# noahares/raxtax

Measured on AMD Instinct MI355X. Metric: classified queries/sec (whole node), higher is better.
Workload: dtype u32 bit-planes + f64

## Files before the change

include/raxtax_hip.h:

```cpp
#ifndef RAXTAX_HIP_H
#define RAXTAX_HIP_H

#include <stddef.h>
#include <stdint.h>

#ifdef __cplusplus
extern "C" {
#endif

#define RTX_ABI_VERSION 6
#define RTX_NUM_KMERS 65536u
#define RTX_MAX_DEPTH 32u

#define RTX_OK 0
#define RTX_ERR_INVALID (-1)
#define RTX_ERR_HIP (-2)
#define RTX_ERR_NO_DEVICE (-3)
#define RTX_ERR_OOM (-4)
#define RTX_ERR_PARSE (-5)
#define RTX_ERR_DEPTH (-6)
#define RTX_ERR_STATE (-7)
#define RTX_ERR_TOO_LONG (-8)
#define RTX_ERR_SENDER (-9)
#define RTX_RETRY_CHUNK 1
// ... 88 lines not shown
#define RTX_OPT_HIT_PAIR 11
#define RTX_OPT_TILE_SKIP 10
#define RTX_OPT_LOCATOR 12
#define RTX_OPT_TILE_PRUNE 13
#define RTX_OPT_FINE_BOUNDS 17
#define RTX_OPT_RECORDS 18
#define RTX_OPT_OVERLAP 19
#define RTX_OPT_MIN_SUB_BATCHES 20
#define RTX_OPT_TWO_LEVEL_BOUNDS 21
#define RTX_OPT_PRUNE_SELF_SAMPLE 22
#define RTX_OPT_RUN_AHEAD 23
#define RTX_OPT_DEVICE_TEXT 24
#define RTX_OPT_STRAND 25
#define RTX_OPT_NEAREST 26
#define RTX_NO_REF 0xFFFFFFFFu
int rtx_index_set_option(rtx_index *index, int option, uint64_t value);

int rtx_index_self_sample(rtx_index *index, const uint8_t *seq_bytes, const uint64_t *seq_off, uint64_t n_refs, uint32_t n_sample, double *live_fraction);
int rtx_index_prune_verdict(const rtx_index *index, int *pruning, double *live_fraction);
int rtx_index_run_ahead_stats(const rtx_index *index, uint64_t *enqueued_ahead, uint64_t *abandoned);
#define RTX_DEFAULT_SEGMENT_CLASSES 1
#define RTX_DEFAULT_EXACT_HASH_MASK 2
int rtx_set_default_option(int option, uint64_t value);

typedef struct {
    uint32_t n_queries;
    uint64_t n_rows;
    const uint32_t *t;
    const uint8_t *status;
    const double *global_signal;
// ... 138 lines not shown
```

raxtax_amd/_build.py:

```python
from __future__ import annotations

import os
import shutil
import subprocess
from pathlib import Path

PKG = Path(__file__).resolve().parent
ROOT = PKG.parent
CSRC = PKG / "csrc"
LIB = PKG / "libraxtax_hip.so"
SOURCES = ["rtx_kernels.hip", "rtx_hit_pair.hip", "rtx_prob_tables.hip", "rtx_cluster.hip", "rtx_segments.hip", "rtx_prune.hip", "rtx_bounds2.hip", "rtx_records.hip", "rtx_finalise.hip", "rtx_text.hip", "rtx_exact.hip", "rtx_strand.hip", "rtx_nearest.hip", "rtx_ingest.hip", "rtx_api_index.hip", "rtx_api_batch.hip", "rtx_api_download.hip", "rtx_api_shard.hip", "rtx_api_debug.hip", "host_tree.cpp", "host_format.cpp", "host_raxtax.cpp", "host_bin.cpp", "host_threads.cpp"]
HEADERS = ["rtx_index.hpp", "rtx_kernels.hpp", "rtx_hit_common.hpp", "rtx_internal.hpp", "rtx_math.hpp", "rtx_wave.hpp", "rtx_walk.hpp", "host_raxtax.hpp"]
CLI = PKG / "raxtax-hip"
SYNTH = PKG / "raxtax-synth"


def _hipcc() -> str:
    for c in (os.environ.get("HIPCC"), shutil.which("hipcc"), "/opt/rocm/bin/hipcc"):
        if c and Path(c).exists():
            return c
    raise RuntimeError("hipcc not found (ROCm toolchain required to build libraxtax_hip.so)")


def _stale(target: Path, deps) -> bool:
    if not target.exists():
        return True
    t = target.stat().st_mtime
# ... 59 lines not shown
```

raxtax_amd/csrc/rtx_api_batch.hip:

```cpp
#include "rtx_index.hpp"

#ifndef RTX_B2_HEAVY_PER_ATILE
#define RTX_B2_HEAVY_PER_ATILE 4u
#endif

namespace rtxi {

int bind(rtx_index *ix) {
    if (!ix) { set_error("null index handle"); return RTX_ERR_INVALID; }
    RTX_HIP(hipSetDevice(ix->device));
    return RTX_OK;
}

int ensure_events(rtx_index *ix, size_t count) {
    while (ix->events.size() < count) {
        hipEvent_t e;
        RTX_HIP(hipEventCreate(&e));
        ix->events.push_back(e);
    }
    return RTX_OK;
}


SubBatch sub_batch_of(rtx_index *ix, uint32_t sb, bool timed) {
// ... 76 lines not shown
    kp.hq = r.d_hq.p;
    kp.t_all = r.d_t_all.p;
    kp.nrows_all = r.d_nrows_all.p;
    kp.hist = sc.d_hist.p;
    kp.hstride = k.hstride;
    return kp;
}

static bool run_prunes(const rtx_index *ix, const rtx_index::BatchClass &k) { return k.prune && !ix->dbg_full_run; }
static bool on_records_path(const rtx_index *ix, const rtx_index::BatchClass &k, const rtx_index::Scratch &sc) { return run_prunes(ix, k) && k.rec && sc.d_rec.p != nullptr; }
static bool on_diet(const rtx_index *ix, const rtx_index::BatchClass &k, const rtx_index::Scratch &sc) { return on_records_path(ix, k, sc) && k.diet && sc.d_cnt_row.p != nullptr; }

static RecordRef record_ref(const rtx_index *ix, const rtx_index::Scratch &sc, const rtx_index::ResultSet &r) { return RecordRef{sc.d_rec_nslots.p, sc.d_rec_slots.p, sc.d_rec_cnt.p, sc.d_rec.p, ix->rec_slots(), ix->rec_seg_len, r.d_flags.p}; }
static ProbTables prob_tables(const rtx_index *ix) { return ProbTables{ix->d_tab_cmf.p, ix->d_tab_ratio.p, ix->d_tab_off.p, ix->d_tab_moff.p, ix->d_tab_ilo.p, ix->d_tab_sat.p, ix->tab_tmax}; }

int enqueue_kmer(rtx_index *ix, const SubBatch &b, hipStream_t s) {
    KmerParams kp = kmer_params(ix, b);
    kp.mode = run_prunes(ix, *b.cls) && ix->seg_blocks ? 1u : 0u;
    if (b.timed_all) RTX_HIP(hipEventRecord(stage_event(ix, b, RTX_STAGE_KMER_EXTRACT, 0), s));
    launch_kmer_extract(s, kp, b.nq);
    if (b.timed_all) RTX_HIP(hipEventRecord(stage_event(ix, b, RTX_STAGE_KMER_EXTRACT, 1), s));
    return RTX_OK;
}

static HitParams hit_params(rtx_index *ix, const SubBatch &b, uint32_t flags) {
    rtx_index::Scratch &sc = ix->sc[b.set];
    rtx_index::ResultSet &r = ix->res();
    const rtx_index::BatchClass &k = *b.cls;
    HitParams hp{};
    hp.bitmap = ix->d_bitmap.p;
    hp.stride_bytes = ix->stride_bytes;
    hp.n_rows1 = ix->n_rows + 1;
    hp.n_refs = ix->n_refs;
    hp.ref_base = ix->ref_lo;
    hp.rows = sc.d_rows.p;
// ... 134 lines not shown
    fp.fine_n_refs = ix->n_refs;
    fp.fine_ref_ntiles = ix->ntiles;
    fp.fine_stats = ix->d_prune_stats.p + 2 * kPruneStatCopies * 8;
    return fp;
}

int enqueue_hit(rtx_index *ix, const SubBatch &b, uint32_t flags, hipStream_t s, int part, hipStream_t s_mid) {
    rtx_index::Scratch &sc = ix->sc[b.set];
    rtx_index::ResultSet &r = ix->res();
    const rtx_index::BatchClass &k = *b.cls;
    ix->last_set = b.set;
    HitParams hp = hit_params(ix, b, flags);
    const bool prune = run_prunes(ix, k);
    if (k.pair && part != 2) {
        if (b.timed_all) RTX_HIP(hipEventRecord(stage_event(ix, b, RTX_STAGE_PAIR_UNION, 0), s));
        launch_pair_union(s, sc.d_rows.p, sc.d_nrows.p, k.rstride, b.nq, sc.d_urec.p, sc.d_nu.p, 2u * k.rstride);
        if (b.timed_all) RTX_HIP(hipEventRecord(stage_event(ix, b, RTX_STAGE_PAIR_UNION, 1), s));
    }
    if (b.timed && !prune) RTX_HIP(hipEventRecord(stage_event(ix, b, RTX_STAGE_HIT_COUNT, 0), s));
    if (part != 0 && !prune) { set_error("internal: a split run without tile pruning"); return RTX_ERR_STATE; }
    if (prune) {
        if (part != 2) {
            const HitParams up = bounds_params(ix, sc, hp);
            if (b.timed) RTX_HIP(hipEventRecord(stage_event(ix, b, RTX_STAGE_TILE_BOUNDS, 0), s));
            ix->two_level_used = part == 0 && ix->two_level_opt && ix->d_abitmap.p && ix->d_bbitmap.p && ix->n_refs == ix->n_total && k.planes <= kBounds2MaxPlanes;
            if (ix->two_level_used) {
                const bool heavy_ok = sc.d_heavy.p && sc.d_heavy_items.p && sc.d_heavy_items.n >= HeavyItemsLayout(b.nq, ix->u_ntiles).total();
                launch_bounds2(s, bounds2_params(ix, sc, up, heavy_ok), b.nq, k.planes, up, ix->u_ntiles, heavy_ok ? sc.d_heavy_items.p : nullptr);
            } else {
                RTX_HIP(hipMemsetAsync(sc.d_best_key.p, 0, (size_t)b.nq * 4, s));
                launch_hit_count_pair_bounds(s, up, b.nq, ix->u_ntiles, k.planes);
// ... 21 lines not shown
        }
        launch_prune(s, pr, prob_tables(ix), b.nq);
        if (part == 1) { RTX_HIP(hipGetLastError()); return RTX_OK; }
        if (part == 0 && ix->fine_opt && ix->d_fbitmap.p && k.pair && sc.d_fine_items.p) {
            const FineItemsLayout fine(b.nq, ix->f_ntiles);
            uint32_t *const fi = sc.d_fine_items.p;
            launch_fine_bounds(s, fine_params(ix, sc, hp), b.nq, ix->ntiles, ix->f_ntiles, pr.pair_live, fine.cursors(fi), fine.items(fi), fine.count(fi), k.planes);
        }
        RTX_HIP(hipMemsetAsync(sc.d_tilemax.p, 0, (size_t)b.nq * ix->ntiles * 2, s));
        hp.live = sc.d_live.p;
        hp.live_words = pr.live_words;
        hp.prune_thr = sc.d_prune_thr.p;
        if (records) hp.rec = rr;
        if (k.pair) {
            const ItemsLayout items(b.nq, ix->ntiles);
            launch_live_items(s, sc.d_live.p, pr.live_words, pr.pair_live, b.nq, ix->ntiles, items.offsets(sc.d_items.p), items.items(sc.d_items.p), items.count(sc.d_items.p));
            hp.items = items.items(sc.d_items.p);
            hp.n_items = items.count(sc.d_items.p);
        }
        if (ix->seg_blocks) {
            KmerParams kp = kmer_params(ix, b);
            kp.mode = 2u;
            kp.live = sc.d_live.p;
            kp.live_words = pr.live_words;
            launch_kmer_extract(s, kp, b.nq);
        }
        if (b.timed) {
            RTX_HIP(hipEventRecord(stage_event(ix, b, RTX_STAGE_TILE_PRUNE, 1), s));
            RTX_HIP(hipEventRecord(stage_event(ix, b, RTX_STAGE_HIT_COUNT, 0), s));
        }
    }
// ... 945 lines not shown
```

raxtax_amd/csrc/rtx_api_index.hip:

```cpp
#include "rtx_index.hpp"

namespace rtx {
int index_device(const rtx_index *index) { return index ? index->device : -1; }
void index_set_shared_device(rtx_index *index, bool shared) { if (index) index->shared_device = shared; }
uint32_t index_swap_min_subs(rtx_index *index, uint32_t v) { if (!index) return 0; const uint32_t old = index->min_subs; index->min_subs = v; return old; }
bool index_strand(const rtx_index *index) { return index && index->strand_opt != 0u; }
bool index_nearest(const rtx_index *index) { return index && index->nearest_opt != 0u; }
bool index_device_text(const rtx_index *index) { return index && index->device_text_opt != 0u; }
uint32_t index_swap_run_ahead(rtx_index *index, uint32_t v) {
    if (!index) return 0;
    const uint32_t old = index->run_ahead_opt;
    (void)rtx_index_set_option(index, RTX_OPT_RUN_AHEAD, v);
    return old;
}
}

namespace {

double statrs_ln_gamma(double x) {
    static const double dk[11] = {2.48574089138753565546e-5, 1.05142378581721974210,  -3.45687097222016235469,
                                  4.51227709466894823700,    -2.98285225323576655721, 1.05639711577126713077,
                                  -1.95428773191645869583e-1, 1.70970543404441224307e-2,
                                  -5.71926117404305781283e-4, 4.63399473359905636708e-6,
                                  -2.71994908488607703910e-9};
// ... 716 lines not shown
        case RTX_OPT_HIT_PAIR:
            index->pair_opt = value ? 1u : 0u;
            return RTX_OK;
        case RTX_OPT_TILE_SKIP:
            index->tile_skip = value ? 1u : 0u;
            return RTX_OK;
        case RTX_OPT_LOCATOR:
            index->locator_opt = value ? 1u : 0u;
            return RTX_OK;
        case RTX_OPT_TILE_PRUNE:
            index->prune_opt = value ? 1u : 0u;
            return RTX_OK;
        case RTX_OPT_FINE_BOUNDS:
            index->fine_opt = value ? 1u : 0u;
            return RTX_OK;
        case RTX_OPT_PRUNE_SELF_SAMPLE:
            index->uploaded = index->ran = index->synced = false;
            index->self_sample_opt = value ? 1u : 0u;
            return RTX_OK;
        case RTX_OPT_RUN_AHEAD:
            index->run_ahead_opt = (uint32_t)std::min<uint64_t>(value, 2u);
            if (!value && index->join_pending) {
                int rc_b = bind(index);
                if (!rc_b) rc_b = settle_join(index);
                return rc_b;
            }
            return RTX_OK;
        case RTX_OPT_DEVICE_TEXT:
            index->device_text_opt = value ? 1u : 0u;
            return RTX_OK;
// ... 52 lines not shown
```

raxtax_amd/csrc/rtx_hit_pair.hip:

```cpp
#include <hip/hip_runtime.h>

#include <algorithm>

#include "rtx_hit_common.hpp"

namespace rtx {

constexpr uint32_t kPairCap = kHitListCap;
constexpr uint32_t kPairListDw = kPairCap + 192u;
constexpr uint32_t kPairMaskWords = 64u;
constexpr uint32_t kPairSidDw = 2u * kSparseIt * 64u;
constexpr uint32_t kPairLdsBytes = 3u * kPairListDw * 4u + 2u * kPairMaskWords * 8u + 32u * 4u + kPairSidDw * 4u;
#ifndef RTX_PAIR_NB
#define RTX_PAIR_NB 3
#endif
#ifndef RTX_PAIR_WAVES
#define RTX_PAIR_WAVES 2
#endif
constexpr int kPairNB = RTX_PAIR_NB;

constexpr uint32_t kUnionMaxRows = 2048u;
__device__ __forceinline__ uint32_t lower_bound_u16(const uint16_t *l, uint32_t n, uint32_t key) {
    uint32_t lo = 0;
#pragma unroll
// ... 268 lines not shown
            asm volatile("" : "+v"(lane_v));
            pair_tile_block<NP, kPacked, kBounds>(p, lds_dw, item / p.ntiles, item % p.ntiles, lane_v);
            wave_lds_sync();
            if (e8 <= g8) break;
            uint32_t nxt = 0;
            if (lane_v == 0u) nxt = atomicAdd(&p.n_items[1u + x], 1u);
            j = first + g8 + (uint32_t)__builtin_amdgcn_readfirstlane((int)nxt);
        }
        return;
    }
    const uint32_t np8 = gridDim.x >> 3;
    const uint32_t pair = blockIdx.x < np8 * 8u ? (blockIdx.x & 7u) * np8 + (blockIdx.x >> 3) : blockIdx.x;
    pair_tile_block<NP, kPacked, kBounds>(p, lds_dw, pair, blockIdx.y, lane);
}

__global__ __launch_bounds__(1024) void live_offsets_kernel(const uint32_t *__restrict__ pair_live, uint32_t np, uint32_t *__restrict__ off,
                                                            uint32_t *__restrict__ n_items) {
    __shared__ uint32_t wsum[2][16];
    const uint32_t tid = threadIdx.x, lane = tid & 63u, wave = tid >> 6;
    constexpr uint32_t kPer = 8;
    uint32_t carry = 0, buf = 0;
    for (uint32_t base = 0; base < np; base += 1024u * kPer, buf ^= 1u) {
        const uint32_t i0 = base + tid * kPer;
        uint32_t c[kPer], cnt = 0;
#pragma unroll
        for (uint32_t j = 0; j < kPer; j++) c[j] = i0 + j < np ? pair_live[i0 + j] : 0u;
#pragma unroll
        for (uint32_t j = 0; j < kPer; j++) cnt += c[j];
        const uint32_t incl = wave_incl_scan_u32(cnt);
        if (lane == 63u) wsum[buf][wave] = incl;
        __syncthreads();
        uint32_t o = carry + incl - cnt, tot = 0;
#pragma unroll
        for (uint32_t w = 0; w < 16u; w++) {
            const uint32_t sw = wsum[buf][w];
            o += w < wave ? sw : 0u;
            tot += sw;
        }
#pragma unroll
        for (uint32_t j = 0; j < kPer; j++) {
            if (i0 + j < np) off[i0 + j] = o;
            o += c[j];
        }
        carry += tot;
    }
    if (tid == 0u) n_items[0] = carry;
    if (tid < 8u) n_items[1u + tid] = 0;
}

__global__ __launch_bounds__(1024) void live_items_kernel(const uint32_t *__restrict__ live, uint32_t live_words, uint32_t nq, uint32_t ntiles,
                                                          const uint32_t *__restrict__ off, uint32_t *__restrict__ items) {
    extern __shared__ uint32_t tl[];
    const uint32_t tid = threadIdx.x, lane = tid & 63u;
    const uint32_t np = (nq + 1u) / 2u, g0 = blockIdx.x * 1024u, pair = g0 + tid;
    for (uint32_t T = tid; T < ntiles; T += 1024) tl[T] = 0;
    __syncthreads();
    const uint32_t nw = (ntiles + 31u) >> 5;
    const bool valid = pair < np;
    const uint32_t *wa = live + (size_t)((valid ? pair : 0u) * 2u) * live_words;
    const bool hb = valid && pair * 2u + 1u < nq;
    if (valid)
        for (uint32_t w = 0; w < nw; w++) {
            uint32_t bits = wa[w] | (hb ? wa[live_words + w] : 0u);
            while (bits) {
                atomicAdd(&tl[w * 32u + (uint32_t)__builtin_ctz(bits)], 1u);
                bits &= bits - 1u;
            }
        }
    __syncthreads();
    if (tid < 64u) {
        uint32_t running = 0;
        for (uint32_t T0 = 0; T0 < ntiles; T0 += 64) {
            const uint32_t v = T0 + lane < ntiles ? tl[T0 + lane] : 0u;
            const uint32_t incl = wave_incl_scan_u32(v);
            if (T0 + lane < ntiles) tl[T0 + lane] = running + incl - v;
            running += (uint32_t)__builtin_amdgcn_readlane((int)incl, 63);
        }
    }
    __syncthreads();
    if (!valid) return;
    const uint32_t base = off[g0];
    for (uint32_t w = 0; w < nw; w++) {
        uint32_t bits = wa[w] | (hb ? wa[live_words + w] : 0u);
        while (bits) {
            const uint32_t tile = w * 32u + (uint32_t)__builtin_ctz(bits);
            bits &= bits - 1u;
            items[base + atomicAdd(&tl[tile], 1u)] = pair * ntiles + tile;
        }
    }
}

void launch_pair_union(hipStream_t s, const uint32_t *rows, const uint32_t *nrows, uint32_t rstride, uint32_t nq, uint2 *urec,
                       uint32_t *nu, uint32_t ustride) {
    hipLaunchKernelGGL(pair_union_kernel, dim3((nq + 1u) / 2u), dim3(64), 0, s, rows, nrows, rstride, nq, urec, nu, ustride);
}

// ... 9 lines not shown
    const dim3 grid = p.items ? dim3((uint32_t)((std::min<uint64_t>((uint64_t)np * ntiles, std::max<uint64_t>((uint64_t)RTX_ITEM_GRID_HALVES * np / 2u, 2048ull)) + 7u) & ~7ull)) : dim3(np, ntiles);
    if (NP <= 10 && p.counts_lo) {
        if (p.items) hipLaunchKernelGGL((hit_count_pair_kernel<(NP <= 10 ? NP : 10), true, false, true>), grid, dim3(64), kPairLdsBytes, s, p);
        else hipLaunchKernelGGL((hit_count_pair_kernel<(NP <= 10 ? NP : 10), true, false, false>), grid, dim3(64), kPairLdsBytes, s, p);
    } else {
        if (p.items) hipLaunchKernelGGL((hit_count_pair_kernel<NP, false, false, true>), grid, dim3(64), kPairLdsBytes, s, p);
        else hipLaunchKernelGGL((hit_count_pair_kernel<NP, false, false, false>), grid, dim3(64), kPairLdsBytes, s, p);
    }
}
void launch_hit_count_pair(hipStream_t s, const HitParams &p, uint32_t nq, uint32_t ntiles, int planes) {
    if (planes <= 8) launch_hit_count_pair_np<8>(s, p, nq, ntiles);
    else if (planes <= 10) launch_hit_count_pair_np<10>(s, p, nq, ntiles);
    else launch_hit_count_pair_np<11>(s, p, nq, ntiles);
}

void launch_live_items(hipStream_t s, const uint32_t *live, uint32_t live_words, const uint32_t *pair_live, uint32_t nq, uint32_t ntiles, uint32_t *off,
                       uint32_t *items, uint32_t *n_items) {
    const uint32_t np = (nq + 1u) / 2u;
    hipLaunchKernelGGL(live_offsets_kernel, dim3(1), dim3(1024), 0, s, pair_live, np, off, n_items);
    hipLaunchKernelGGL(live_items_kernel, dim3((np + 1023u) / 1024u), dim3(1024), (size_t)ntiles * 4, s, live, live_words, nq, ntiles, off, items);
}

void launch_hit_count_pair_bounds(hipStream_t s, const HitParams &p, uint32_t nq, uint32_t u_ntiles, int planes) {
    if (planes <= 8) hipLaunchKernelGGL((hit_count_pair_kernel<8, true, 1, false>), dim3((nq + 1u) / 2u, u_ntiles), dim3(64), kPairLdsBytes, s, p);
    else if (planes <= 10) hipLaunchKernelGGL((hit_count_pair_kernel<10, true, 1, false>), dim3((nq + 1u) / 2u, u_ntiles), dim3(64), kPairLdsBytes, s, p);
    else hipLaunchKernelGGL((hit_count_pair_kernel<11, false, 1, false>), dim3((nq + 1u) / 2u, u_ntiles), dim3(64), kPairLdsBytes, s, p);
}

void launch_hit_count_pair_bounds_items(hipStream_t s, const HitParams &p, uint32_t nq, uint32_t u_ntiles, int planes) {
    const uint32_t np = (nq + 1u) / 2u;
    const dim3 grid((uint32_t)((std::min<uint64_t>((uint64_t)np * u_ntiles, 4096ull) + 7u) & ~7ull));
    if (planes <= 8) hipLaunchKernelGGL((hit_count_pair_kernel<8, true, 1, true>), grid, dim3(64), kPairLdsBytes, s, p);
    else if (planes <= 10) hipLaunchKernelGGL((hit_count_pair_kernel<10, true, 1, true>), grid, dim3(64), kPairLdsBytes, s, p);
    else hipLaunchKernelGGL((hit_count_pair_kernel<11, false, 1, true>), grid, dim3(64), kPairLdsBytes, s, p);
}
// ... 77 lines not shown
```

raxtax_amd/csrc/rtx_index.hpp:

```cpp
#pragma once

#include <hip/hip_runtime.h>

#include <algorithm>
#include <cmath>
#include <cstdlib>
#include <cstring>
#include <thread>

#include "rtx_internal.hpp"
#include "rtx_kernels.hpp"
#include "rtx_math.hpp"

using namespace rtx;

namespace rtxi {


constexpr uint32_t kEmptyRow = 0xFFFFFFFFu;
constexpr uint32_t kLnFactLen = 98320;

#define RTX_HIP(call)                                                                          \
    do {                                                                                       \
        hipError_t e_ = (call);                                                                \
// ... 148 lines not shown
    uint32_t pair_opt = 1;
    uint32_t prune_opt = 1;
    uint32_t self_sample_opt = 1;
    bool prune_pays = true;
    double self_live = -1.0;
    bool pruning() const { return prune_opt != 0u && (prune_pays || self_sample_opt == 0u); }
    bool dbg_full = false;
    bool dbg_full_run = false;
    DevBuf<uint32_t> d_ubitmap;
    uint32_t u_stride_bytes = 0, u_ntiles = 0;
    uint64_t u_nblocks = 0;
    DevBuf<uint32_t> d_fbitmap;
    uint32_t f_stride_bytes = 0, f_ntiles = 0;
    uint64_t f_nblocks = 0;
    uint32_t fine_opt = 1;
    DevBuf<uint32_t> d_abitmap;
    DevBuf<uint8_t> d_bbitmap;
    uint32_t n_atiles = 0, n_btiles = 0;
    DevBuf<uint8_t> d_cbitmap;
    uint32_t two_level_opt = 1;
    uint32_t b2_delta[4] = {283u, 205u, 92u, 128u};
    bool two_level_used = false;
    uint32_t rec_seg_len = 1024;
    uint32_t diet_shift = 3;
    uint32_t rec_opt = 4;
    uint32_t rec_slots() const { return std::min<uint32_t>(rec_opt, kRecMaxSlots); }
    uint32_t overlap_opt = 1;
    uint32_t overlap_used = 0;
    hipStream_t stream2 = nullptr, stream3 = nullptr, hit_stream = nullptr;
    std::vector<hipEvent_t> ev_front, ev_back, ev_mid;
// ... 255 lines not shown
int alloc_final(rtx_index *ix, rtx_index::ResultSet &r, uint64_t n_queries);
int enqueue_finalise(rtx_index *ix, const SubBatch &b, hipStream_t s);
int enqueue_text(rtx_index *ix, const rtx_index::ResultSet &r);


struct ItemList {
    size_t np, ntiles;
    ItemList(size_t nq, size_t tiles) : np((nq + 1u) / 2u), ntiles(tiles) {}
    size_t cap() const { return np * ntiles; }
    size_t end() const { return cap() + 9u; }
    uint32_t *items(uint32_t *p) const { return p; }
    uint32_t *count(uint32_t *p) const { return p + cap(); }
};
struct ItemsLayout : ItemList {
    using ItemList::ItemList;
    size_t total() const { return end() + 2u * np; }
    uint32_t *pair_live(uint32_t *p) const { return p + end(); }
    uint32_t *offsets(uint32_t *p) const { return p + end() + np; }
};
struct FineItemsLayout : ItemList {
    using ItemList::ItemList;
    size_t total() const { return end() + ntiles; }
    uint32_t *cursors(uint32_t *p) const { return p + end(); }
};
struct HeavyItemsLayout : ItemList {
    using ItemList::ItemList;
    size_t total() const { return end(); }
};
struct LiveLayout {
    uint32_t ntiles;
    uint32_t words() const { return (ntiles + 31u) / 32u + 1u; }
    size_t total(size_t B) const { return (B + 1u) * words(); }
};
// ... 66 lines not shown
```

raxtax_amd/csrc/rtx_kernels.hip:

```cpp
#include <hip/hip_runtime.h>

#include "rtx_kernels.hpp"
#include "rtx_math.hpp"
#include "rtx_wave.hpp"
#include "rtx_hit_common.hpp"
#include "rtx_walk.hpp"

namespace rtx {

static constexpr uint32_t kEmptyRow = 0xFFFFFFFFu;

__global__ __launch_bounds__(256) void bitmap_build_kernel(const uint64_t *__restrict__ off,
                                                           const uint32_t *__restrict__ post,
                                                           const uint32_t *__restrict__ row_of,
                                                           uint32_t *__restrict__ bitmap, uint32_t stride_words, uint32_t n_rows1,
                                                           uint32_t ref_lo, uint32_t ref_hi, uint32_t shift) {
    const uint32_t k = blockIdx.x;
    const uint32_t row = row_of[k];
    if (row == kEmptyRow) return;
    const uint64_t b = off[k], e = off[k + 1];
    for (uint64_t i = b + threadIdx.x; i < e; i += blockDim.x) {
        const uint32_t g = post[i];
        if (g < ref_lo || g >= ref_hi) continue;
        uint32_t word, bit;
// ... 96 lines not shown

    uint32_t t = 0, nrows = 0;
    unsigned long long hq = 0;
    uint32_t *rout = p.rows + (size_t)q * p.rstride;
    const unsigned long long lt_mask = (1ull << lane) - 1ull;
    if (mode == 2u) {
        nrows = p.nrows[q];
    } else {
    for (uint32_t i = lane; i < 2048; i += 64) bm[i] = 0;
    {
        uint32_t *h = p.hist + (size_t)q * p.hstride;
        for (uint32_t i = lane; i < p.hstride; i += 64) h[i] = 0;
    }
    __syncthreads();

    if (len >= 8) {
        const uint64_t nwin = len - 7;
        const uint64_t wpl = (nwin + 63) / 64;
        const uint64_t w0 = (uint64_t)lane * wpl;
        const uint64_t w1 = w0 + wpl < nwin ? w0 + wpl : nwin;
        for (uint64_t i = w0; i < w1; i += 16) {
            unsigned long long v[3];
            __builtin_memcpy(v, seq + i, 24);
            const uint32_t nw = w1 - i < 16 ? (uint32_t)(w1 - i) : 16u;
            uint32_t k = 0, run = 0;
#pragma unroll
            for (int b = 0; b < 23; b++) {
                const uint32_t c = (uint32_t)(v[b >> 3] >> ((b & 7) * 8)) & 0xFFu;
                const bool ok = c == 1u || c == 2u || c == 4u || c == 8u;
                k = ((k << 2) | (((uint32_t)__ffs((int)c) - 1u) & 3u)) & 0xFFFFu;
                run = ok ? run + 1u : 0u;
                if (b >= 7 && (uint32_t)(b - 7) < nw && run >= 8u) atomicOr(&bm[k >> 5], 1u << (k & 31u));
            }
        }
    }
    __syncthreads();

    uint16_t *kout = p.kmers + (size_t)q * p.kstride;
    const unsigned long long *bm64 = reinterpret_cast<const unsigned long long *>(bm);
    uint32_t base = 0;
    for (uint32_t r = 0; r < 16; r++) {
        unsigned long long word = bm64[r * 64 + lane];
        const uint32_t cnt = (uint32_t)__popcll(word);
        const uint32_t incl = wave_incl_scan_u32(cnt);
        uint32_t pos = base + incl - cnt;
        const uint32_t kbase = (r * 64 + lane) * 64;
        while (word) {
            const uint32_t bit = (uint32_t)__builtin_ctzll(word);
            word &= word - 1;
            if (pos < p.kstride) kout[pos] = (uint16_t)(kbase + bit);
// ... 905 lines not shown
```

raxtax_amd/csrc/rtx_kernels.hpp:

```cpp
#pragma once

#include <hip/hip_runtime.h>

#include <cstdint>

#include "raxtax_hip.h"

namespace rtx {

#ifndef RTX_NODE_TYPES_DEFINED
#define RTX_NODE_TYPES_DEFINED
enum NodeType : uint8_t { kInner = 0, kTaxon = 1, kSequence = 2 };
#endif

constexpr uint32_t kWalkMaxRows = 208;
constexpr uint32_t kSegSlotEntries = 16, kSegSparseMax = 16, kSegMaxSparseRows = 255;
constexpr uint32_t kSegPad = 8192;
__host__ __device__ inline uint32_t seg_pad(uint32_t i) { return kSegPad + ((i & 63u) << 2); }
constexpr uint32_t kKmerFewLive = 8;
constexpr uint32_t kHitListCap = 1024;

struct DevRow {
    uint32_t node;
    uint8_t k[RTX_MAX_DEPTH];
// ... 387 lines not shown
    WalkParams walk;
    unsigned long long *prefix_stats;
    unsigned long long *stats;
};
void launch_records_tail(hipStream_t s, const TailParams &p, uint32_t nq);

void launch_bitmap_build(hipStream_t s, const uint64_t *off, const uint32_t *post, const uint32_t *row_of,
                         uint32_t *bitmap, uint32_t stride_words, uint32_t n_rows1, uint32_t ref_lo, uint32_t ref_hi, uint32_t shift = 0);
void launch_ref_kmer_mark(hipStream_t s, const uint8_t *bases, const uint64_t *off, uint64_t n_refs, uint32_t *present);
void launch_ref_bitmap_set(hipStream_t s, const uint8_t *bases, const uint64_t *off, uint64_t n_refs,
                           const uint32_t *row_of, uint32_t *bitmap, uint32_t stride_words, uint32_t n_rows1, uint32_t shift = 0);
void launch_row_len_pack(hipStream_t s, const uint32_t *row_of, const uint32_t *list_len, uint2 *out);
void launch_row_popcount(hipStream_t s, const uint32_t *row_of, const uint32_t *bitmap, uint32_t stride_words, uint32_t n_rows1,
                         uint32_t *list_len);
void launch_kmer_extract(hipStream_t s, const KmerParams &p, uint32_t nq);
void launch_hit_count(hipStream_t s, const HitParams &p, uint32_t nq, uint32_t ntiles, int planes);
void launch_pair_union(hipStream_t s, const uint32_t *rows, const uint32_t *nrows, uint32_t rstride, uint32_t nq, uint2 *urec,
                       uint32_t *nu, uint32_t ustride);
void launch_hit_count_pair(hipStream_t s, const HitParams &p, uint32_t nq, uint32_t ntiles, int planes);
void launch_live_items(hipStream_t s, const uint32_t *live, uint32_t live_words, const uint32_t *pair_live, uint32_t nq, uint32_t ntiles, uint32_t *off,
                       uint32_t *items, uint32_t *n_items);
void launch_hit_count_pair_bounds(hipStream_t s, const HitParams &p, uint32_t nq, uint32_t u_ntiles, int planes);
void launch_hit_count_pair_bounds_items(hipStream_t s, const HitParams &p, uint32_t nq, uint32_t u_ntiles, int planes);
void launch_fine_bounds(hipStream_t s, const HitParams &p, uint32_t nq, uint32_t ntiles, uint32_t f_ntiles, uint32_t *pair_live, uint32_t *cnt,
                        uint32_t *items, uint32_t *n_items, int planes);
size_t prob_table_lds_bytes(uint32_t tmax);
void launch_prob_table(hipStream_t s, const ProbParams &p, uint32_t nq);
size_t prob_lookup_lds_bytes(uint32_t tmax);
void launch_prob_tables_build(hipStream_t s, const ProbTables &tb, const double *lf, const double *inv);
void launch_prob_order(hipStream_t s, const uint32_t *t, uint32_t nq, uint32_t *order);
void launch_prob_lookup(hipStream_t s, const ProbParams &p, const ProbTables &tb, uint32_t nq);
void launch_seg_popcount(hipStream_t s, const uint32_t *bitmap, uint32_t stride_bytes, uint32_t n_rows1, uint32_t ntiles, uint16_t *pop);
void launch_seg_emit(hipStream_t s, const uint32_t *bitmap, uint32_t stride_bytes, uint32_t n_rows1, uint32_t ntiles,
                     const uint32_t *seginfo, uint32_t seg_stride, uint16_t *slots);
void launch_sketch(hipStream_t s, const uint8_t *bases, const uint64_t *off, uint32_t n_q, uint64_t *keys, uint32_t *idx);
// ... 20 lines not shown
```

Baseline: 13.07 million.

## Fuse k-mer extraction with pair union lists and merge live-items offset pass

Adds a pair_extract kernel that builds the k-mer sets of both queries in a pair within one block and emits their per-query row lists and the merged union records together, so the separate pair_union pass is skipped on the pruned pair path. It also folds the single-block live-offsets scan into the live-items kernel, where each block recomputes its prefix by summing all earlier pair_live entries. This removes one or two kernel launches and a re-read of row lists, at the cost of a lower-occupancy 128-thread extract kernel and prefix work that grows with block index. The fused path is enabled by default behind a new option.

Result: no change. 12.95 million (-0.9%).

```diff
diff --git a/include/raxtax_hip.h b/include/raxtax_hip.h
--- a/include/raxtax_hip.h
+++ b/include/raxtax_hip.h
@@ -126,6 +126,7 @@
 #define RTX_OPT_STRAND 25
 #define RTX_OPT_NEAREST 26
 #define RTX_NO_REF 0xFFFFFFFFu
+#define RTX_OPT_PAIR_LISTS 27
 int rtx_index_set_option(rtx_index *index, int option, uint64_t value);
 
 int rtx_index_self_sample(rtx_index *index, const uint8_t *seq_bytes, const uint64_t *seq_off, uint64_t n_refs, uint32_t n_sample, double *live_fraction);
diff --git a/raxtax_amd/_build.py b/raxtax_amd/_build.py
--- a/raxtax_amd/_build.py
+++ b/raxtax_amd/_build.py
@@ -9,8 +9,8 @@
 ROOT = PKG.parent
 CSRC = PKG / "csrc"
 LIB = PKG / "libraxtax_hip.so"
-SOURCES = ["rtx_kernels.hip", "rtx_hit_pair.hip", "rtx_prob_tables.hip", "rtx_cluster.hip", "rtx_segments.hip", "rtx_prune.hip", "rtx_bounds2.hip", "rtx_records.hip", "rtx_finalise.hip", "rtx_text.hip", "rtx_exact.hip", "rtx_strand.hip", "rtx_nearest.hip", "rtx_ingest.hip", "rtx_api_index.hip", "rtx_api_batch.hip", "rtx_api_download.hip", "rtx_api_shard.hip", "rtx_api_debug.hip", "host_tree.cpp", "host_format.cpp", "host_raxtax.cpp", "host_bin.cpp", "host_threads.cpp"]
-HEADERS = ["rtx_index.hpp", "rtx_kernels.hpp", "rtx_hit_common.hpp", "rtx_internal.hpp", "rtx_math.hpp", "rtx_wave.hpp", "rtx_walk.hpp", "host_raxtax.hpp"]
+SOURCES = ["rtx_kernels.hip", "rtx_hit_pair.hip", "rtx_pair_extract.hip", "rtx_prob_tables.hip", "rtx_cluster.hip", "rtx_segments.hip", "rtx_prune.hip", "rtx_bounds2.hip", "rtx_records.hip", "rtx_finalise.hip", "rtx_text.hip", "rtx_exact.hip", "rtx_strand.hip", "rtx_nearest.hip", "rtx_ingest.hip", "rtx_api_index.hip", "rtx_api_batch.hip", "rtx_api_download.hip", "rtx_api_shard.hip", "rtx_api_debug.hip", "host_tree.cpp", "host_format.cpp", "host_raxtax.cpp", "host_bin.cpp", "host_threads.cpp"]
+HEADERS = ["rtx_index.hpp", "rtx_kernels.hpp", "rtx_hit_common.hpp", "rtx_internal.hpp", "rtx_math.hpp", "rtx_wave.hpp", "rtx_kmer_set.hpp", "rtx_walk.hpp", "host_raxtax.hpp"]
 CLI = PKG / "raxtax-hip"
 SYNTH = PKG / "raxtax-synth"
 
diff --git a/raxtax_amd/csrc/rtx_api_batch.hip b/raxtax_amd/csrc/rtx_api_batch.hip
--- a/raxtax_amd/csrc/rtx_api_batch.hip
+++ b/raxtax_amd/csrc/rtx_api_batch.hip
@@ -114,11 +114,20 @@
 static RecordRef record_ref(const rtx_index *ix, const rtx_index::Scratch &sc, const rtx_index::ResultSet &r) { return RecordRef{sc.d_rec_nslots.p, sc.d_rec_slots.p, sc.d_rec_cnt.p, sc.d_rec.p, ix->rec_slots(), ix->rec_seg_len, r.d_flags.p}; }
 static ProbTables prob_tables(const rtx_index *ix) { return ProbTables{ix->d_tab_cmf.p, ix->d_tab_ratio.p, ix->d_tab_off.p, ix->d_tab_moff.p, ix->d_tab_ilo.p, ix->d_tab_sat.p, ix->tab_tmax}; }
 
+static bool fused_pair_lists(const rtx_index *ix, const rtx_index::BatchClass &k) {
+    return ix->pair_lists_opt != 0u && k.pair && run_prunes(ix, k) && ix->seg_blocks != 0u && ix->n_refs == ix->n_total;
+}
+
 int enqueue_kmer(rtx_index *ix, const SubBatch &b, hipStream_t s) {
     KmerParams kp = kmer_params(ix, b);
     kp.mode = run_prunes(ix, *b.cls) && ix->seg_blocks ? 1u : 0u;
     if (b.timed_all) RTX_HIP(hipEventRecord(stage_event(ix, b, RTX_STAGE_KMER_EXTRACT, 0), s));
-    launch_kmer_extract(s, kp, b.nq);
+    if (fused_pair_lists(ix, *b.cls)) {
+        rtx_index::Scratch &sc = ix->sc[b.set];
+        launch_pair_extract(s, kp, b.nq, sc.d_urec.p, sc.d_nu.p, 2u * b.cls->rstride);
+    } else {
+        launch_kmer_extract(s, kp, b.nq);
+    }
     if (b.timed_all) RTX_HIP(hipEventRecord(stage_event(ix, b, RTX_STAGE_KMER_EXTRACT, 1), s));
     return RTX_OK;
 }
@@ -283,7 +292,7 @@
     const bool prune = run_prunes(ix, k);
     if (k.pair && part != 2) {
         if (b.timed_all) RTX_HIP(hipEventRecord(stage_event(ix, b, RTX_STAGE_PAIR_UNION, 0), s));
-        launch_pair_union(s, sc.d_rows.p, sc.d_nrows.p, k.rstride, b.nq, sc.d_urec.p, sc.d_nu.p, 2u * k.rstride);
+        if (!fused_pair_lists(ix, k)) launch_pair_union(s, sc.d_rows.p, sc.d_nrows.p, k.rstride, b.nq, sc.d_urec.p, sc.d_nu.p, 2u * k.rstride);
         if (b.timed_all) RTX_HIP(hipEventRecord(stage_event(ix, b, RTX_STAGE_PAIR_UNION, 1), s));
     }
     if (b.timed && !prune) RTX_HIP(hipEventRecord(stage_event(ix, b, RTX_STAGE_HIT_COUNT, 0), s));
@@ -335,7 +344,7 @@
         if (records) hp.rec = rr;
         if (k.pair) {
             const ItemsLayout items(b.nq, ix->ntiles);
-            launch_live_items(s, sc.d_live.p, pr.live_words, pr.pair_live, b.nq, ix->ntiles, items.offsets(sc.d_items.p), items.items(sc.d_items.p), items.count(sc.d_items.p));
+            launch_live_items(s, sc.d_live.p, pr.live_words, pr.pair_live, b.nq, ix->ntiles, items.items(sc.d_items.p), items.count(sc.d_items.p));
             hp.items = items.items(sc.d_items.p);
             hp.n_items = items.count(sc.d_items.p);
         }
diff --git a/raxtax_amd/csrc/rtx_api_index.hip b/raxtax_amd/csrc/rtx_api_index.hip
--- a/raxtax_amd/csrc/rtx_api_index.hip
+++ b/raxtax_amd/csrc/rtx_api_index.hip
@@ -754,6 +754,10 @@
         case RTX_OPT_FINE_BOUNDS:
             index->fine_opt = value ? 1u : 0u;
             return RTX_OK;
+        case RTX_OPT_PAIR_LISTS:
+            if (value > 1) break;
+            index->pair_lists_opt = (uint32_t)value;
+            return RTX_OK;
         case RTX_OPT_PRUNE_SELF_SAMPLE:
             index->uploaded = index->ran = index->synced = false;
             index->self_sample_opt = value ? 1u : 0u;
diff --git a/raxtax_amd/csrc/rtx_hit_pair.hip b/raxtax_amd/csrc/rtx_hit_pair.hip
--- a/raxtax_amd/csrc/rtx_hit_pair.hip
+++ b/raxtax_amd/csrc/rtx_hit_pair.hip
@@ -306,47 +306,29 @@
     pair_tile_block<NP, kPacked, kBounds>(p, lds_dw, pair, blockIdx.y, lane);
 }
 
-__global__ __launch_bounds__(1024) void live_offsets_kernel(const uint32_t *__restrict__ pair_live, uint32_t np, uint32_t *__restrict__ off,
-                                                            uint32_t *__restrict__ n_items) {
+__global__ __launch_bounds__(1024) void live_items_kernel(const uint32_t *__restrict__ live, uint32_t live_words, uint32_t nq, uint32_t ntiles,
+                                                          const uint32_t *__restrict__ pair_live, uint32_t *__restrict__ items,
+                                                          uint32_t *__restrict__ n_items) {
+    extern __shared__ uint32_t tl[];
     __shared__ uint32_t wsum[2][16];
-    const uint32_t tid = threadIdx.x, lane = tid & 63u, wave = tid >> 6;
-    constexpr uint32_t kPer = 8;
-    uint32_t carry = 0, buf = 0;
-    for (uint32_t base = 0; base < np; base += 1024u * kPer, buf ^= 1u) {
-        const uint32_t i0 = base + tid * kPer;
-        uint32_t c[kPer], cnt = 0;
-#pragma unroll
-        for (uint32_t j = 0; j < kPer; j++) c[j] = i0 + j < np ? pair_live[i0 + j] : 0u;
-#pragma unroll
-        for (uint32_t j = 0; j < kPer; j++) cnt += c[j];
-        const uint32_t incl = wave_incl_scan_u32(cnt);
-        if (lane == 63u) wsum[buf][wave] = incl;
-        __syncthreads();
-        uint32_t o = carry + incl - cnt, tot = 0;
-#pragma unroll
-        for (uint32_t w = 0; w < 16u; w++) {
-            const uint32_t sw = wsum[buf][w];
-            o += w < wave ? sw : 0u;
-            tot += sw;
-        }
-#pragma unroll
-        for (uint32_t j = 0; j < kPer; j++) {
-            if (i0 + j < np) off[i0 + j] = o;
-            o += c[j];
-        }
-        carry += tot;
-    }
-    if (tid == 0u) n_items[0] = carry;
-    if (tid < 8u) n_items[1u + tid] = 0;
-}
-
-__global__ __launch_bounds__(1024) void live_items_kernel(const uint32_t *__restrict__ live, uint32_t live_words, uint32_t nq, uint32_t ntiles,
-                                                          const uint32_t *__restrict__ off, uint32_t *__restrict__ items) {
-    extern __shared__ uint32_t tl[];
     const uint32_t tid = threadIdx.x, lane = tid & 63u;
     const uint32_t np = (nq + 1u) / 2u, g0 = blockIdx.x * 1024u, pair = g0 + tid;
     for (uint32_t T = tid; T < ntiles; T += 1024) tl[T] = 0;
+    uint32_t before = 0;
+    for (uint32_t i = tid; i < g0; i += 1024u) before += pair_live[i];
+    uint32_t own = pair < np ? pair_live[pair < np ? pair : 0u] : 0u;
+#pragma unroll
+    for (int d = 32; d >= 1; d >>= 1) {
+        before += __shfl_xor(before, d, 64);
+        own += __shfl_xor(own, d, 64);
+    }
+    if (lane == 0u) { wsum[0][tid >> 6] = before; wsum[1][tid >> 6] = own; }
     __syncthreads();
+    uint32_t base = 0, group = 0;
+#pragma unroll
+    for (uint32_t w = 0; w < 16u; w++) { base += wsum[0][w]; group += wsum[1][w]; }
+    if (blockIdx.x == 0u && tid < 8u) n_items[1u + tid] = 0;
+    if (blockIdx.x == gridDim.x - 1u && tid == 0u) n_items[0] = base + group;
     const uint32_t nw = (ntiles + 31u) >> 5;
     const bool valid = pair < np;
     const uint32_t *wa = live + (size_t)((valid ? pair : 0u) * 2u) * live_words;
@@ -371,7 +353,6 @@
     }
     __syncthreads();
     if (!valid) return;
-    const uint32_t base = off[g0];
     for (uint32_t w = 0; w < nw; w++) {
         uint32_t bits = wa[w] | (hb ? wa[live_words + w] : 0u);
         while (bits) {
@@ -411,11 +392,10 @@
     else launch_hit_count_pair_np<11>(s, p, nq, ntiles);
 }
 
-void launch_live_items(hipStream_t s, const uint32_t *live, uint32_t live_words, const uint32_t *pair_live, uint32_t nq, uint32_t ntiles, uint32_t *off,
+void launch_live_items(hipStream_t s, const uint32_t *live, uint32_t live_words, const uint32_t *pair_live, uint32_t nq, uint32_t ntiles,
                        uint32_t *items, uint32_t *n_items) {
     const uint32_t np = (nq + 1u) / 2u;
-    hipLaunchKernelGGL(live_offsets_kernel, dim3(1), dim3(1024), 0, s, pair_live, np, off, n_items);
-    hipLaunchKernelGGL(live_items_kernel, dim3((np + 1023u) / 1024u), dim3(1024), (size_t)ntiles * 4, s, live, live_words, nq, ntiles, off, items);
+    hipLaunchKernelGGL(live_items_kernel, dim3((np + 1023u) / 1024u), dim3(1024), (size_t)ntiles * 4, s, live, live_words, nq, ntiles, pair_live, items, n_items);
 }
 
 void launch_hit_count_pair_bounds(hipStream_t s, const HitParams &p, uint32_t nq, uint32_t u_ntiles, int planes) {
diff --git a/raxtax_amd/csrc/rtx_index.hpp b/raxtax_amd/csrc/rtx_index.hpp
--- a/raxtax_amd/csrc/rtx_index.hpp
+++ b/raxtax_amd/csrc/rtx_index.hpp
@@ -186,6 +186,10 @@
     uint32_t f_stride_bytes = 0, f_ntiles = 0;
     uint64_t f_nblocks = 0;
     uint32_t fine_opt = 1;
+#ifndef RTX_PAIR_LISTS_DEFAULT
+#define RTX_PAIR_LISTS_DEFAULT 1
+#endif
+    uint32_t pair_lists_opt = RTX_PAIR_LISTS_DEFAULT;
     DevBuf<uint32_t> d_abitmap;
     DevBuf<uint8_t> d_bbitmap;
     uint32_t n_atiles = 0, n_btiles = 0;
@@ -471,9 +475,8 @@
 };
 struct ItemsLayout : ItemList {
     using ItemList::ItemList;
-    size_t total() const { return end() + 2u * np; }
+    size_t total() const { return end() + np; }
     uint32_t *pair_live(uint32_t *p) const { return p + end(); }
-    uint32_t *offsets(uint32_t *p) const { return p + end() + np; }
 };
 struct FineItemsLayout : ItemList {
     using ItemList::ItemList;
diff --git a/raxtax_amd/csrc/rtx_kernels.hip b/raxtax_amd/csrc/rtx_kernels.hip
--- a/raxtax_amd/csrc/rtx_kernels.hip
+++ b/raxtax_amd/csrc/rtx_kernels.hip
@@ -3,6 +3,7 @@
 #include "rtx_kernels.hpp"
 #include "rtx_math.hpp"
 #include "rtx_wave.hpp"
+#include "rtx_kmer_set.hpp"
 #include "rtx_hit_common.hpp"
 #include "rtx_walk.hpp"
 
@@ -134,26 +135,7 @@
     }
     __syncthreads();
 
-    if (len >= 8) {
-        const uint64_t nwin = len - 7;
-        const uint64_t wpl = (nwin + 63) / 64;
-        const uint64_t w0 = (uint64_t)lane * wpl;
-        const uint64_t w1 = w0 + wpl < nwin ? w0 + wpl : nwin;
-        for (uint64_t i = w0; i < w1; i += 16) {
-            unsigned long long v[3];
-            __builtin_memcpy(v, seq + i, 24);
-            const uint32_t nw = w1 - i < 16 ? (uint32_t)(w1 - i) : 16u;
-            uint32_t k = 0, run = 0;
-#pragma unroll
-            for (int b = 0; b < 23; b++) {
-                const uint32_t c = (uint32_t)(v[b >> 3] >> ((b & 7) * 8)) & 0xFFu;
-                const bool ok = c == 1u || c == 2u || c == 4u || c == 8u;
-                k = ((k << 2) | (((uint32_t)__ffs((int)c) - 1u) & 3u)) & 0xFFFFu;
-                run = ok ? run + 1u : 0u;
-                if (b >= 7 && (uint32_t)(b - 7) < nw && run >= 8u) atomicOr(&bm[k >> 5], 1u << (k & 31u));
-            }
-        }
-    }
+    kmer_set_build(bm, seq, len, lane);
     __syncthreads();
 
     uint16_t *kout = p.kmers + (size_t)q * p.kstride;
diff --git a/raxtax_amd/csrc/rtx_kernels.hpp b/raxtax_amd/csrc/rtx_kernels.hpp
--- a/raxtax_amd/csrc/rtx_kernels.hpp
+++ b/raxtax_amd/csrc/rtx_kernels.hpp
@@ -425,11 +425,12 @@
 void launch_row_popcount(hipStream_t s, const uint32_t *row_of, const uint32_t *bitmap, uint32_t stride_words, uint32_t n_rows1,
                          uint32_t *list_len);
 void launch_kmer_extract(hipStream_t s, const KmerParams &p, uint32_t nq);
+void launch_pair_extract(hipStream_t s, const KmerParams &p, uint32_t nq, uint2 *urec, uint32_t *nu, uint32_t ustride);
 void launch_hit_count(hipStream_t s, const HitParams &p, uint32_t nq, uint32_t ntiles, int planes);
 void launch_pair_union(hipStream_t s, const uint32_t *rows, const uint32_t *nrows, uint32_t rstride, uint32_t nq, uint2 *urec,
                        uint32_t *nu, uint32_t ustride);
 void launch_hit_count_pair(hipStream_t s, const HitParams &p, uint32_t nq, uint32_t ntiles, int planes);
-void launch_live_items(hipStream_t s, const uint32_t *live, uint32_t live_words, const uint32_t *pair_live, uint32_t nq, uint32_t ntiles, uint32_t *off,
+void launch_live_items(hipStream_t s, const uint32_t *live, uint32_t live_words, const uint32_t *pair_live, uint32_t nq, uint32_t ntiles,
                        uint32_t *items, uint32_t *n_items);
 void launch_hit_count_pair_bounds(hipStream_t s, const HitParams &p, uint32_t nq, uint32_t u_ntiles, int planes);
 void launch_hit_count_pair_bounds_items(hipStream_t s, const HitParams &p, uint32_t nq, uint32_t u_ntiles, int planes);
diff --git a/raxtax_amd/csrc/rtx_kmer_set.hpp b/raxtax_amd/csrc/rtx_kmer_set.hpp
--- /dev/null
+++ b/raxtax_amd/csrc/rtx_kmer_set.hpp
@@ -0,0 +1,32 @@
+#pragma once
+
+#include <hip/hip_runtime.h>
+
+#include <cstdint>
+
+namespace rtx {
+
+__device__ __forceinline__ void kmer_set_build(uint32_t *bm, const uint8_t *__restrict__ seq, uint64_t len, uint32_t lane) {
+    if (len >= 8) {
+        const uint64_t nwin = len - 7;
+        const uint64_t wpl = (nwin + 63) / 64;
+        const uint64_t w0 = (uint64_t)lane * wpl;
+        const uint64_t w1 = w0 + wpl < nwin ? w0 + wpl : nwin;
+        for (uint64_t i = w0; i < w1; i += 16) {
+            unsigned long long v[3];
+            __builtin_memcpy(v, seq + i, 24);
+            const uint32_t nw = w1 - i < 16 ? (uint32_t)(w1 - i) : 16u;
+            uint32_t k = 0, run = 0;
+#pragma unroll
+            for (int b = 0; b < 23; b++) {
+                const uint32_t c = (uint32_t)(v[b >> 3] >> ((b & 7) * 8)) & 0xFFu;
+                const bool ok = c == 1u || c == 2u || c == 4u || c == 8u;
+                k = ((k << 2) | (((uint32_t)__ffs((int)c) - 1u) & 3u)) & 0xFFFFu;
+                run = ok ? run + 1u : 0u;
+                if (b >= 7 && (uint32_t)(b - 7) < nw && run >= 8u) atomicOr(&bm[k >> 5], 1u << (k & 31u));
+            }
+        }
+    }
+}
+
+}
diff --git a/raxtax_amd/csrc/rtx_pair_extract.hip b/raxtax_amd/csrc/rtx_pair_extract.hip
--- /dev/null
+++ b/raxtax_amd/csrc/rtx_pair_extract.hip
@@ -0,0 +1,171 @@
+#include <hip/hip_runtime.h>
+
+#include "rtx_kernels.hpp"
+#include "rtx_wave.hpp"
+#include "rtx_kmer_set.hpp"
+
+namespace rtx {
+
+static constexpr uint32_t kEmptyRow = 0xFFFFFFFFu;
+constexpr uint32_t kPxListCap = 4096u;
+
+__device__ __forceinline__ uint32_t wave_total_u32(uint32_t v) { return (uint32_t)__builtin_amdgcn_readlane((int)wave_incl_scan_u32(v), 63); }
+
+__global__ __launch_bounds__(128) void pair_extract_kernel(KmerParams p, uint32_t nq, uint2 *__restrict__ urec, uint32_t *__restrict__ nu,
+                                                           uint32_t ustride) {
+    __shared__ __attribute__((aligned(16))) uint32_t bm[2][2048];
+    __shared__ uint16_t ulist[kPxListCap];
+    __shared__ uint32_t xcnt[2][2][4];
+    __shared__ unsigned long long xhq[2][2];
+    const uint32_t pair = blockIdx.x, lane = threadIdx.x & 63u;
+    const uint32_t wave = (uint32_t)__builtin_amdgcn_readfirstlane((int)(threadIdx.x >> 6));
+    const uint32_t q = pair * 2u + wave;
+    const bool have = q < nq;
+    const uint64_t gq = p.q0 + q;
+    uint64_t len = 0;
+    const uint8_t *seq = p.bases;
+    if (have) {
+        const uint64_t qin = p.perm[gq];
+        const uint64_t b0 = p.base_off[qin];
+        len = p.base_off[qin + 1] - b0;
+        seq = p.bases + b0;
+    }
+    for (uint32_t i = lane; i < 2048; i += 64) bm[wave][i] = 0;
+    if (have) {
+        uint32_t *h = p.hist + (size_t)q * p.hstride;
+        for (uint32_t i = lane; i < p.hstride; i += 64) h[i] = 0;
+    }
+    __syncthreads();
+    kmer_set_build(bm[wave], seq, len, lane);
+    __syncthreads();
+
+    const unsigned long long *sa = reinterpret_cast<const unsigned long long *>(bm[0]), *sb = reinterpret_cast<const unsigned long long *>(bm[1]);
+    uint32_t ha[2] = {0, 0}, hb[2] = {0, 0}, hu[2] = {0, 0};
+#pragma unroll
+    for (uint32_t r = 0; r < 16; r++) {
+        const unsigned long long a = sa[r * 64 + lane], b = sb[r * 64 + lane];
+        ha[r >> 3] += (uint32_t)__popcll(a);
+        hb[r >> 3] += (uint32_t)__popcll(b);
+        hu[r >> 3] += (uint32_t)__popcll(a | b);
+    }
+    const uint32_t a0 = wave_total_u32(ha[0]), b0n = wave_total_u32(hb[0]), u0 = wave_total_u32(hu[0]);
+    const uint32_t t_a = a0 + wave_total_u32(ha[1]), t_b = b0n + wave_total_u32(hb[1]), n_list = u0 + wave_total_u32(hu[1]);
+    {
+        uint16_t *ka = p.kmers + (size_t)(pair * 2u) * p.kstride, *kb = ka + p.kstride;
+        uint32_t base_a = wave ? a0 : 0u, base_b = wave ? b0n : 0u, base_u = wave ? u0 : 0u;
+        for (uint32_t r = wave * 8u; r < wave * 8u + 8u; r++) {
+            const unsigned long long a = sa[r * 64 + lane], b = sb[r * 64 + lane];
+            unsigned long long u = a | b;
+            const uint32_t ca = (uint32_t)__popcll(a), cb = (uint32_t)__popcll(b), cu = (uint32_t)__popcll(u);
+            const uint32_t ia = wave_incl_scan_u32(ca), ib = wave_incl_scan_u32(cb), iu = wave_incl_scan_u32(cu);
+            uint32_t pos_a = base_a + ia - ca, pos_b = base_b + ib - cb, pos_u = base_u + iu - cu;
+            const uint32_t kbase = (r * 64 + lane) * 64;
+            while (u) {
+                const uint32_t bit = (uint32_t)__builtin_ctzll(u);
+                u &= u - 1;
+                const uint16_t k = (uint16_t)(kbase + bit);
+                if (pos_u < kPxListCap) ulist[pos_u] = k;
+                pos_u++;
+                if ((a >> bit) & 1ull) {
+                    if (pos_a < p.kstride) ka[pos_a] = k;
+                    pos_a++;
+                }
+                if ((b >> bit) & 1ull) {
+                    if (pos_b < p.kstride) kb[pos_b] = k;
+                    pos_b++;
+                }
+            }
+            base_a += (uint32_t)__builtin_amdgcn_readlane((int)ia, 63);
+            base_b += (uint32_t)__builtin_amdgcn_readlane((int)ib, 63);
+            base_u += (uint32_t)__builtin_amdgcn_readlane((int)iu, 63);
+        }
+    }
+    __syncthreads();
+
+    const uint32_t n_l = n_list < kPxListCap ? n_list : kPxListCap;
+    const unsigned long long lt_mask = (1ull << lane) - 1ull;
+    uint32_t *ra = p.rows + (size_t)(pair * 2u) * p.rstride, *rb = ra + p.rstride;
+    uint2 *out = urec + (size_t)pair * ustride;
+    uint32_t n_a = 0, n_b = 0, n_u = 0;
+    unsigned long long hq_a = 0, hq_b = 0;
+    for (uint32_t i0 = 0, turn = 0; i0 < n_l; i0 += 512, turn ^= 1u) {
+        uint32_t kk[4], row[4], ll[4];
+        bool in_a[4], in_b[4];
+#pragma unroll
+        for (int u = 0; u < 4; u++) {
+            const uint32_t i = i0 + wave * 256u + (uint32_t)u * 64u + lane;
+            kk[u] = i < n_l ? (uint32_t)ulist[i] : 0xFFFFFFFFu;
+        }
+#pragma unroll
+        for (int u = 0; u < 4; u++) {
+            const uint32_t k = kk[u] & 0xFFFFu;
+            in_a[u] = kk[u] != 0xFFFFFFFFu && ((bm[0][k >> 5] >> (k & 31u)) & 1u);
+            in_b[u] = kk[u] != 0xFFFFFFFFu && ((bm[1][k >> 5] >> (k & 31u)) & 1u);
+        }
+#pragma unroll
+        for (int u = 0; u < 4; u++) {
+            row[u] = kEmptyRow;
+            ll[u] = 0;
+            if (kk[u] != 0xFFFFFFFFu) {
+                const uint2 rl = p.row_len[kk[u]];
+                row[u] = rl.x;
+                ll[u] = rl.y;
+            }
+        }
+        uint32_t la[4], lb[4], lu[4], c_a = 0, c_b = 0, c_u = 0;
+#pragma unroll
+        for (int u = 0; u < 4; u++) {
+            hq_a += in_a[u] ? ll[u] : 0u;
+            hq_b += in_b[u] ? ll[u] : 0u;
+            const bool sv = row[u] != kEmptyRow;
+            const unsigned long long m_a = __ballot(sv && in_a[u]), m_b = __ballot(sv && in_b[u]), m_u = __ballot(sv);
+            la[u] = c_a + (uint32_t)__popcll(m_a & lt_mask);
+            lb[u] = c_b + (uint32_t)__popcll(m_b & lt_mask);
+            lu[u] = c_u + (uint32_t)__popcll(m_u & lt_mask);
+            c_a += (uint32_t)__popcll(m_a);
+            c_b += (uint32_t)__popcll(m_b);
+            c_u += (uint32_t)__popcll(m_u);
+        }
+        if (lane == 0) { xcnt[turn][wave][0] = c_a; xcnt[turn][wave][1] = c_b; xcnt[turn][wave][2] = c_u; }
+        __syncthreads();
+        const uint32_t o_a = xcnt[turn][wave ^ 1u][0], o_b = xcnt[turn][wave ^ 1u][1], o_u = xcnt[turn][wave ^ 1u][2];
+        const uint32_t f_a = n_a + (wave ? o_a : 0u), f_b = n_b + (wave ? o_b : 0u), f_u = n_u + (wave ? o_u : 0u);
+#pragma unroll
+        for (int u = 0; u < 4; u++) {
+            if (row[u] == kEmptyRow) continue;
+            const uint32_t pa = f_a + la[u], pb = f_b + lb[u], pu = f_u + lu[u];
+            if (in_a[u] && pa < p.rstride) ra[pa] = row[u];
+            if (in_b[u] && pb < p.rstride) rb[pb] = row[u];
+            if (pu < ustride)
+                out[pu] = make_uint2((row[u] & 0xFFFFu) | ((uint32_t)in_a[u] << 30) | ((uint32_t)in_b[u] << 31),
+                                     (in_a[u] ? pa : 0xFFFFu) | ((in_b[u] ? pb : 0xFFFFu) << 16));
+        }
+        n_a += c_a + o_a;
+        n_b += c_b + o_b;
+        n_u += c_u + o_u;
+    }
+#pragma unroll
+    for (int d = 32; d >= 1; d >>= 1) {
+        hq_a += __shfl_xor(hq_a, d, 64);
+        hq_b += __shfl_xor(hq_b, d, 64);
+    }
+    if (lane == 0) { xhq[wave][0] = hq_a; xhq[wave][1] = hq_b; }
+    __syncthreads();
+    if (!have) return;
+    const uint32_t nrows = wave ? n_b : n_a, t = wave ? t_b : t_a;
+    uint32_t *rout = wave ? rb : ra;
+    for (uint32_t i = nrows + lane; i < ((nrows + 63u) & ~63u) && i < p.rstride; i += 64) rout[i] = p.zero_row;
+    if (lane == 0) {
+        p.t[q] = t > 65535u ? 0u : t;
+        p.nrows[q] = nrows;
+        p.hq[gq] = xhq[0][wave] + xhq[1][wave];
+        p.t_all[gq] = t;
+        if (wave == 0u) nu[pair] = n_u;
+    }
+}
+
+void launch_pair_extract(hipStream_t s, const KmerParams &p, uint32_t nq, uint2 *urec, uint32_t *nu, uint32_t ustride) {
+    hipLaunchKernelGGL(pair_extract_kernel, dim3((nq + 1u) / 2u), dim3(128), 0, s, p, nq, urec, nu, ustride);
+}
+
+}
```
